# yinan-codes/Rossby-wave-ray-tracing

Hardware: AMD Instinct MI355X
Metric: ray-steps/sec (whole node), 10^6 rays RKF45; max |Δpos| vs CPU ref (higher is better)
Workload: dtype f64

## Files before the change

rossby-wave-ray-tracing_amd/csrc/ray_point.h:

```cpp
#ifndef RWRT_RAY_POINT_H
#define RWRT_RAY_POINT_H

#include <hip/hip_runtime.h>

#include <cmath>
#include <cstdint>

#include "rwrt.h"
#include "nproots.h"

#ifndef RARE
#define RARE(c) (c)
#endif

namespace rwrt {

constexpr double kPi = 3.14159265358979323846;
constexpr double kHalfPi = 0.5 * kPi;
constexpr double kTwoPi = 2.0 * kPi;
constexpr double kNaN = __builtin_nan("");

__device__ __forceinline__ void div2(double a1, double b1, double a2, double b2, double& qa,
                                     double& qb) {
  double dA, dB, rA, rB, eA, eB, nA, nB;
// ... 67 lines not shown
struct Field {
  const double* __restrict__ P;
  int W, H;
  double lon0, dlon, lat0, dlat;
};

struct Corners {
  const double* a;
  const double* b;
  const double* c;
  const double* d;
  double wa, wb, wc, wd;
  unsigned key_x, key_y;
  unsigned pa, pb, pc, pd;
  unsigned oa, ob, oc, od;
};

__device__ __forceinline__ Corners corners(const Field& F, double lon, double lat) {
  const double lons = py_mod_2pi_again(lon);
  double x, y;
  div2(lons - F.lon0, F.dlon, lat - F.lat0, F.dlat, x, y);
  const int ix = floor_i32(x), iy = floor_i32(y);
  const int x0 = clip(ix, F.W - 1), x1 = clip(inc_i32(ix), F.W - 1);
  const int y0 = clip(iy, F.H - 1), y1 = clip(inc_i32(iy), F.H - 1);
  const double sx = x - (double)x0, sy = y - (double)y0;
  const unsigned c0 = __umul24(x0, F.H), c1 = __umul24(x1, F.H);
  Corners k;
  k.pa = c0 + y1;
  k.pb = c1 + y1;
  k.pc = c0 + y0;
  k.pd = c1 + y0;
  k.oa = __umul24(k.pa, kNF);
  k.ob = __umul24(k.pb, kNF);
  k.oc = __umul24(k.pc, kNF);
  k.od = __umul24(k.pd, kNF);
  k.a = F.P + k.oa;
  k.b = F.P + k.ob;
  k.c = F.P + k.oc;
  k.d = F.P + k.od;
  k.wa = (1.0 - sx) * sy;
  k.wb = sx * sy;
  k.wc = (1.0 - sx) * (1.0 - sy);
// ... 136 lines not shown
```

rossby-wave-ray-tracing_amd/csrc/rwrt.hip:

```cpp

#include <hip/hip_runtime.h>

#include <cmath>
#include <cstdint>
#include <cstdlib>
#include <cstdio>
#include <cstring>
#include <mutex>
#include <string>
#include <type_traits>

#include "rwrt.h"
#include "nproots.h"

#ifdef RWRT_ANALYZE_HOT
__device__ __forceinline__ bool rwrt_rare_sink(bool c) {
  asm volatile("; rare %0" ::"s"(__builtin_amdgcn_ballot_w64(c)));
  return false;
}
#define RARE(c) rwrt_rare_sink(c)
#else
#define RARE(c) (c)
#endif
#ifdef RWRT_ANALYZE_MARK
// ... 64 lines not shown
  return (ab >= 0x1p-100 && ab <= 0x1p100) ? r : 0.0;
}
__device__ __forceinline__ double div_hw(double a, double b, double rb) {
  const double q = a * rb;
  const double rem = fma(-b, q, a);
  double r = copysign(fma(rem, rb, q), q);
  const double aa = fabs(a);
  const bool bad = !(aa < 0x1p600) | ((aa < 0x1p-900) & (aa != 0.0)) | (rb == 0.0);
  if (RARE(bad)) {
    asm volatile("");
    r = a / b;
  }
  return r;
}

__constant__ int kRefIndex[11] = {0, 1, 2, 3, 4, 5, 6, 7, 8, 9, 11};

struct StaticBG {
  static constexpr bool kTimeVarying = false;
  Field F;
  const char* img = nullptr;
  __device__ __forceinline__ void interp11(double lon, double lat, double, double g[11]) const {
    rwrt::interp11(F, py_mod_2pi(lon), lat, g);
  }
  __device__ __forceinline__ void interp4(double lon, double lat, double, double& fu, double& fv,
                                          double& fqx, double& fqy) const {
    rwrt::interp4(F, py_mod_2pi(lon), lat, fu, fv, fqx, fqy);
  }
};

struct PendingPoint {
  double lon, lat, t;
};
template <class BG>
__device__ __forceinline__ PendingPoint lookup_begin(const BG&, double lon, double lat, double t) {
  return PendingPoint{lon, lat, t};
}
template <class BG>
__device__ __forceinline__ void lookup_end(const BG& B, const PendingPoint& p, double g[11]) {
  B.interp11(p.lon, p.lat, p.t, g);
}

constexpr int kCacheChunks = 4 * 6;
constexpr int kCacheBytesPerWave = kCacheChunks * 64 * 16;
// ... 4 lines not shown
  typedef __attribute__((address_space(3))) char lds_char;
  unsigned b = (unsigned)(size_t)(lds_char*)wave_base;
  asm volatile("" : "+s"(b));
  return (char*)(lds_char*)(size_t)b;
}

__device__ __forceinline__ void lds_dma_wait() { asm volatile("s_waitcnt vmcnt(0)" ::: "memory"); }

constexpr int kCacheAhead = 1;
static_assert(kCacheAhead >= 0 && kCacheAhead < 4, "end() prologue waits for chunks 0-3 only");

constexpr unsigned kImgTile = 6 * 1024;
inline size_t cache_image_bytes(int64_t npts) { return (size_t)((npts + 63) / 64) * kImgTile; }
__device__ __forceinline__ unsigned img_offset(unsigned p) { return __umul24(p >> 6, kImgTile - 1024u) + p * 16u; }

__global__ void cache_image_kernel(Field F, char* __restrict__ img) {
  const int64_t n = (int64_t)F.W * F.H * 6;
  for (int64_t i = blockIdx.x * (int64_t)blockDim.x + threadIdx.x; i < n; i += (int64_t)gridDim.x * blockDim.x) {
    const unsigned p = (unsigned)(i / 6), q = (unsigned)(i - (int64_t)p * 6);
    const double2 v = reinterpret_cast<const double2*>(F.P + (size_t)p * kNF)[q];
    *reinterpret_cast<double2*>(img + img_offset(p) + q * 1024u) = v;
  }
}

struct CachedStaticBG {
  static constexpr bool kTimeVarying = false;
  Field F;
  const char* img;
  char* wave_base;
  const char* img_hi;
  unsigned lane16;
  mutable unsigned key_x, key_y;

  struct Pending {
    double wa, wb, wc, wd;
  };
  __device__ __forceinline__ const double2& chunk(int j, int q) const {
    return *reinterpret_cast<const double2*>(wave_base + (j * 6 + q) * 1024 + lane16);
  }
  __device__ __forceinline__ void refill(unsigned o0, unsigned o1, unsigned o2, unsigned o3) const {
    typedef __attribute__((address_space(3))) char lds_char;
    const unsigned l = (unsigned)(size_t)(lds_char*)wave_base;
    unsigned keep;
#define RWRT_REFILL_LO(O, LOFF)                                                  \
    "s_add_u32 m0, %[l], " #LOFF "\n\t"                                          \
    "s_nop 0\n\t"                                                               \
    "global_load_lds_dwordx4 %[" #O "], %[g0]\n\t"                              \
    "global_load_lds_dwordx4 %[" #O "], %[g0] offset:1024\n\t"                  \
    "global_load_lds_dwordx4 %[" #O "], %[g0] offset:2048\n\t"                  \
    "global_load_lds_dwordx4 %[" #O "], %[g0] offset:3072\n\t"
// ... 49 lines not shown
    if (k.key_x != key_x || k.key_y != key_y) {
      quad_refill(img_offset(k.pa), img_offset(k.pb), img_offset(k.pc), img_offset(k.pd), qa, qb);
      key_x = k.key_x;
      key_y = k.key_y;
    }
    return Pending{k.wa, k.wb, k.wc, k.wd};
  }
  __device__ __forceinline__ Pending begin(double lon, double lat) const {
    const Corners k = corners(F, py_mod_2pi(lon), lat);
    const bool miss = k.key_x != key_x || k.key_y != key_y;
    if (miss) {
      refill(img_offset(k.pa), img_offset(k.pb), img_offset(k.pc), img_offset(k.pd));
      key_x = k.key_x;
      key_y = k.key_y;
    }
    return Pending{k.wa, k.wb, k.wc, k.wd};
  }
  template <class Fill>
  __device__ __forceinline__ void end(const Pending& p, double g[11], Fill&& fill) const {
    asm volatile("s_waitcnt vmcnt(8)" ::: "memory");
    Corners k;
    k.wa = p.wa;
    k.wb = p.wb;
    k.wc = p.wc;
    k.wd = p.wd;
    constexpr int kAhead = kCacheAhead;
    double2 v[6][4];
#pragma unroll
    for (int q = 0; q <= kAhead; ++q)
#pragma unroll
      for (int j = 0; j < 4; ++j) v[q][j] = chunk(j, q);
// ... 10 lines not shown
        if (n == 4) lds_dma_wait();
#pragma unroll
        for (int j = 0; j < 4; ++j) v[n][j] = chunk(j, n);
      }
      __builtin_amdgcn_sched_barrier(0);
    }
  }
  __device__ __forceinline__ void interp4(double lon, double lat, double, double& fu, double& fv,
                                          double& fqx, double& fqy) const {
    rwrt::interp4(F, py_mod_2pi(lon), lat, fu, fv, fqx, fqy);
  }
};
__device__ __forceinline__ CachedStaticBG::Pending lookup_begin(const CachedStaticBG& B, double lon,
                                                                double lat, double) {
  return B.begin(lon, lat);
}
__device__ __forceinline__ void lookup_end(const CachedStaticBG& B,
                                           const CachedStaticBG::Pending& p, double g[11]) {
  B.end(p, g, [] {});
}
template <class Fill>
__device__ __forceinline__ void lookup_end(const CachedStaticBG& B, const CachedStaticBG::Pending& p,
                                           double g[11], Fill&& fill) {
  B.end(p, g, fill);
}
template <class BG, class Fill>
__device__ __forceinline__ void lookup_end(const BG& B, const typename std::decay<decltype(lookup_begin(
                                                            B, 0.0, 0.0, 0.0))>::type& p,
                                           double g[11], Fill&& fill) {
  fill();
// ... 694 lines not shown
}
__device__ __forceinline__ void ugvg(double fu, double fv, double fqx, double fqy,
                                     const KapTerms& w, double& ug, double& vg) {
  const double kap = w.kap, kap2 = w.kap2, denom = w.denom;
  double qu, qv;
  div2(((1.0 - kap2) * fqy) - ((2.0 * kap) * fqx), denom,
       ((2.0 * kap) * fqy) + ((1.0 - kap2) * fqx), denom, qu, qv);
  ug = fu + qu;
  vg = fv + qv;
}
__device__ __forceinline__ void ugvg(double fu, double fv, double fqx, double fqy,
                                     double k, double l, double& ug, double& vg) {
  ugvg(fu, fv, fqx, fqy, kap_terms(k, l), ug, vg);
}

__device__ __forceinline__ double rcp2(double d) {
  double r = __builtin_amdgcn_rcp(d);
  double e = fma(-d, r, 1.0);
  r = fma(r, e, r);
  e = fma(-d, r, 1.0);
  return fma(r, e, r);
}
__device__ __forceinline__ double qdiv(double n, double d, double r) {
  const double q = n * r;
  const double e = fma(-d, q, n);
  return __builtin_amdgcn_div_fixup(fma(e, r, q), d, n);
}
struct DivGuard {
  int nlo = 0, nhi = 0, dlo = 0, dhi = 0;
  __device__ __forceinline__ void num(double n) {
    const int e = __builtin_amdgcn_frexp_exp(n);
    nlo = ::min(nlo, e);
    nhi = ::max(nhi, e);
  }
  __device__ __forceinline__ void den(double d) {
    const int e = __builtin_amdgcn_frexp_exp(d);
    dlo = ::min(dlo, e);
    dhi = ::max(dhi, e);
  }
  __device__ __forceinline__ bool ok() const {
    return (nlo >= -899) & (nhi <= 600) & (dlo >= -99) & (dhi <= 100);
  }
// ... 65 lines not shown
  const double dzwn = (-kx) * ((fmux + kap * fmvx) + qk);
  const double dmwn = (-kx) * ((fmuy + kap * fmvy) + ql);
  const double damp1 = qdiv(2.0 * ((fmux + fmvy) + kap * (fmvx + fmuy)), kw.kap1, kw.rk1, G);
  const double damp2 = qdiv(2.0 * (kap * (fmqxx - fmqyy) + (kap2 - 1.0) * fmqxy), kw.denom, kw.rden, G);
  const double damp3 = (-2.0 * s) * fmv;
  const double damp = (damp1 + damp2) + damp3;
  const double rR = rcp2(kREarth);
  dy[0] = qdiv(ug, kREarth, rR, G);
  dy[1] = qdiv(vg * c, kREarth, rR, G);
  dy[2] = qdiv(dzwn, kREarth, rR, G);
  dy[3] = qdiv(dmwn, kREarth, rR, G);
  dy[4] = qdiv(damp * amp, kREarth, rR, G);
  return G.ok() & (M.m == 1.0);
}

__device__ __forceinline__ bool rhs_tail_fast_pair(const double g[11], const Merc& M, double s, double c,
                                                   double tn, double kx, const KapTermsR& kw, DivGuard G,
                                                   double amp, bool up, double& dA, double& dB, double& dC,
                                                   double& ug, double& vg) {
  const double fu = g[F_U], fv = g[F_V];
  const double rc = rcp2(c);
  const double fmuy = g[F_UY] + tn * fu, fmvy = g[F_VY] + tn * fv;
  const double fmqx = g[F_QX], fmqy = g[F_QY] * c, fmqxx = g[F_QXX];
  const double fmqyx = g[F_QXY] * c, fmqxy = fmqyx;
  const double fmqyy = ((g[F_QYY] * c) - (g[F_QY] * s)) * c;
  const double kap = kw.kap, kap2 = kw.kap2;
  const double fmu = qdiv(fu, c, rc, G), fmv = qdiv(fv, c, rc, G);
  const double fmux = qdiv(g[F_UX], c, rc, G), fmvx = qdiv(g[F_VX], c, rc, G);
  ug = fmu + qdiv(((1.0 - kap2) * fmqy) - ((2.0 * kap) * fmqx), kw.denom, kw.rden, G);
  vg = fmv + qdiv(((2.0 * kap) * fmqy) + ((1.0 - kap2) * fmqx), kw.denom, kw.rden, G);
// ... 1 lines not shown
  const double ql = qdiv(kap * fmqxy - fmqyy, kw.kk, kw.rkk, G);
  const double dzwn = (-kx) * ((fmux + kap * fmvx) + qk);
  const double dmwn = (-kx) * ((fmuy + kap * fmvy) + ql);
  const double damp1 = qdiv(2.0 * ((fmux + fmvy) + kap * (fmvx + fmuy)), kw.kap1, kw.rk1, G);
  const double damp2 = qdiv(2.0 * (kap * (fmqxx - fmqyy) + (kap2 - 1.0) * fmqxy), kw.denom, kw.rden, G);
  const double damp3 = (-2.0 * s) * fmv;
  const double damp = (damp1 + damp2) + damp3;
  const double rR = rcp2(kREarth);
  const double vgc = vg * c;
  dA = qdiv(up ? vgc : ug, kREarth, rR, G);
  dB = qdiv(up ? dmwn : dzwn, kREarth, rR, G);
  dC = qdiv(damp * amp, kREarth, rR, G);
  return G.ok() & (M.m == 1.0);
}

template <class BG>
__device__ __forceinline__ void ray_rhs(const BG& B, double t, const double* y, double* dy,
                                        double* aux = nullptr) {
  const double lon = y[0], lat = y[1], kx = y[2];
  const bool bad = fabs(lat) >= kHalfPi || fabs(y[3]) >= 100.0;
  const double ky = bad ? kNaN : y[3], amp = y[4];
  double g[11];
  MARK("r_entry");
  const auto trig = np_math::nm_sincostan_begin(lat);
  MARK("r_trig_begin");
  double s, c;
  DivGuard G;
  KapTermsR kw;
  const auto pending = lookup_begin(B, lon, lat, t);
  MARK("r_lookup_begin");
  double tn;
  np_math::nm_sincostan_end(lat, trig, s, c, tn);
  MARK("r_trig_end");
  __builtin_amdgcn_sched_barrier(0);
  lookup_end(B, pending, g, [&] { kw = kap_terms_r(kx, ky, G); MARK("r_kap"); });
  MARK("r_lookup_end");
  const Merc M = merc_factors(lat, c, s);
  double ug, vg;
  if (RARE(!rhs_tail_fast(g, M, s, c, tn, kx, kw, G, amp, dy, ug, vg))) {
    asm volatile("");
    rhs_tail_ieee(g, M, s, c, tn, kx, ky, amp, dy, ug, vg);
  }
  MARK("r_tail");
  if (aux) {
    aux[0] = ug;
    aux[1] = vg;
    aux[2] = bad ? kNaN : c;
  }
}

#ifndef RWRT_TEAM_SINORCOS
#define RWRT_TEAM_SINORCOS 1
#endif

template <class Lookup>
__device__ __forceinline__ void ray_rhs_f32(Lookup&& lookup, const double* y, double* dy, double* aux) {
  const double lat = y[1];
  const bool bad = fabs(lat) >= kHalfPi || fabs(y[3]) >= 100.0;
  const float fnan = __builtin_nanf("");
  const float kx = (float)y[2], ky = bad ? fnan : (float)y[3], amp = (float)y[4];
  float g[11];
  lookup(g);
  if (!(fabs(lat) <= kHalfPi)) {
// ... 592 lines not shown
__global__ void mercator_kernel(Field F, int64_t n, const double* __restrict__ lon,
                                const double* __restrict__ lat, double* __restrict__ out) {
  nm_stage<NM_SINCOS | NM_TAN>();
  for (int64_t i = blockIdx.x * (int64_t)blockDim.x + threadIdx.x; i < n;
       i += (int64_t)gridDim.x * blockDim.x) {
    const double la = lat[i];
    double g[11], o[12];
    interp11(F, py_mod_2pi(lon[i]), la, g);
    const Merc M = merc_factors(la, k_cos(la), k_sin(la));
    mercator12(g, M, k_tan(la), o);
#pragma unroll
    for (int q = 0; q < 12; ++q) out[q * n + i] = o[q];
  }
}

__global__ void rhs_kernel(Field F, int64_t n, const double* __restrict__ y,
                           double* __restrict__ dydt) {
  nm_stage<NM_SINCOS | NM_TAN>();
  for (int64_t i = blockIdx.x * (int64_t)blockDim.x + threadIdx.x; i < n;
       i += (int64_t)gridDim.x * blockDim.x) {
    double yy[5], d[5];
#pragma unroll
    for (int v = 0; v < 5; ++v) yy[v] = y[v * n + i];
    ray_rhs(StaticBG{F}, 0.0, yy, d);
#pragma unroll
    for (int v = 0; v < 5; ++v) dydt[v * n + i] = d[v];
  }
}

__global__ void attempt_kernel(Field F, int64_t n, const double* __restrict__ y,
                               const double* __restrict__ f, const double* __restrict__ h,
                               double rtol, double atol, double* __restrict__ Kout,
                               double* __restrict__ ynew, double* __restrict__ err) {
  nm_stage<NM_SINCOS | NM_TAN>();
  const RayProblem P{StaticBG{F}};
  for (int64_t i = blockIdx.x * (int64_t)blockDim.x + threadIdx.x; i < n;
       i += (int64_t)gridDim.x * blockDim.x) {
    double yy[5], ff[5], yn[5], k6[5];
#pragma unroll
// ... 527 lines not shown
  using type = BlockVaryingBG<T>;
};

template <class BG, class LBG, bool kTrace, bool kReplica, bool kPair = false>
__device__ __forceinline__ void run_rays(const RunArgs<BG>& a, const LBG& lbg, char* smem, int64_t hw) {
  using RayProblem = RayProblemT<LBG>;
  const RayProblem P{lbg};
  const bool writer = kReplica ? (threadIdx.x & 63u) == 0 : kPair ? (threadIdx.x & 63u) < 32u : true;
  Lane<RayProblem, KStore> L;
  L.K.p = reinterpret_cast<double*>(smem) + threadIdx.x;
  L.K.stride = 256;
  int64_t ray = -1, nacc = 0, nrej = 0;
  double* rows = nullptr;
  int32_t it = 0, nanrow = 0, wpos = 0;
  double prev_lon = 0.0, prev_lat = 0.0, cos_prev = 0.0;
  constexpr bool kHandoff = std::is_same<LBG, CachedStaticBG>::value && !kReplica && !kPair && !kTrace;
  bool handoff = false;
  __builtin_amdgcn_s_setprio(1);
  for (;;) {
    if (ray < 0) {
      int64_t w;
      if (kReplica) {
        if (hw < 0) break;
        w = hw;
        hw = -1;
      } else if (kPair) {
        int64_t w0 = 0;
        if ((threadIdx.x & 63u) < 32u) w0 = a.n_heavy + atomicAdd(&a.queue[1], 1);
        w = __shfl(w0, (int)(threadIdx.x & 31u));
      } else {
        w = a.n_heavy + atomicAdd(&a.queue[1], 1);
// ... 139 lines not shown
      if (q < nq) {
        CachedStaticBG QB = lbg;
        QB.key_x = QB.key_y = ~0u;
        QuadRole R;
        R.role = threadIdx.x & 3;
        R.odd = (R.role & 1) != 0;
        R.high = (R.role & 2) != 0;
        KQuad K{reinterpret_cast<double*>(smem) + threadIdx.x};
        quad_run<false>(a, QB, R, K, qray, qrows, y, f, aux, qt, qhabs, qhs, qnacc, qnrej, 0, qnanrow, qit,
                        qplon, qplat, qcos, (qflags & 1) != 0, (qflags & 2) != 0, 0);
      }
    }
  }
}

template <class BG, bool kTrace = false>
__global__ void __launch_bounds__(256, 1) __attribute__((aligned(RWRT_RUN_ALIGN)))
rk45_run_kernel(RunArgs<BG> a) {
  nm_stage<NM_ALL>();
  constexpr int kKBytes = 5 * 5 * 256 * 8;
  __shared__ __attribute__((aligned(16))) char smem[kKBytes + LaneBG<BG>::kLdsBytes];
  if constexpr (std::is_same<BG, StaticBG>::value) {
    const int lb = (int)blockIdx.x;
#ifdef RWRT_ANALYZE_QUAD
    if (true) {
#else
    if (RARE(lb < a.heavy_blocks)) {
#endif
      __builtin_amdgcn_s_setprio(1);
      quad_rays<kTrace>(a, smem + kKBytes, reinterpret_cast<double*>(smem), lb);
      return;
    }
  }
// ... 4 lines not shown
      using BBG = typename TvBlock<BG>::type;
      run_rays<BG, BBG, false, true>(a, BBG::make(a.B, smem + kKBytes), smem, w);
      return;
    }
  }
  if constexpr (std::is_same<BG, VaryingBG<double>>::value) {
#ifdef RWRT_ANALYZE_PAIR
    if (true) {
#else
    if (a.B.half) {
#endif
      run_rays<BG, PairVaryingBG64, false, false, true>(a, PairVaryingBG64::make(a.B, smem + kKBytes), smem, -1);
      return;
    }
  }
  run_rays<BG, typename LaneBG<BG>::type, kTrace, false>(a, LaneBG<BG>::make(a.B, smem + kKBytes), smem, -1);
}

__global__ void frozen_flag_kernel(const double* __restrict__ state, int64_t nray,
                                   uint8_t* __restrict__ frozen, int32_t* __restrict__ tail_from = nullptr,
                                   int32_t it_begin = 0, int32_t it_end = 0) {
  for (int64_t i = blockIdx.x * (int64_t)blockDim.x + threadIdx.x; i < nray;
       i += (int64_t)gridDim.x * blockDim.x) {
    double sum = state[i];
#pragma unroll
    for (int v = 1; v < 5; ++v) sum = sum + state[v * nray + i];
    const bool frz = isnan(sum / 5.0);
    frozen[i] = frz ? 1 : 0;
    if (tail_from) tail_from[i] = frz ? it_begin : it_end;
  }
}
// ... 114 lines not shown
    case 26: r = np_math::nm_cos(a); break;
    case 27: r = np_math::nm_tan(a); break;
    case 28: r = np_math::nm_pow(a, b); break;
    case 29: r = np_math::nm_rcp14(a); break;
    case 30: { double sn, cs, tn; k_sincostan(a, sn, cs, tn); r = sn; } break;
    case 31: { double sn, cs, tn; k_sincostan(a, sn, cs, tn); r = cs; } break;
    case 32: { double sn, cs, tn; k_sincostan(a, sn, cs, tn); r = tn; } break;
    case 33: r = k_pow(a, b); break;
    case 34: r = qdiv(a, b, rcp2(b)); break;
    case 35: {
      DivGuard G;
      G.num(a);
      G.den(b);
      r = G.ok() ? 1.0 : 0.0;
    } break;
    default: r = kNaN; break;
  }
  out[i] = r;
}

__device__ __forceinline__ bool rhs_bad(const double* y) {
  return fabs(y[1]) >= kHalfPi || fabs(y[3]) >= 100.0;
}

struct Rk4Args {
  Field F;
  const char* img;
  int64_t nray;
  double dt, cut_off;
  int32_t nt, it_begin, it_end;
// ... 342 lines not shown
rwrt_status ctx_flags(rwrt_ctx* c, int64_t nray) {
  if ((size_t)nray <= c->cap) return RWRT_OK;
  if (c->flags) {
    if ((c->used && hipEventSynchronize(c->done) != hipSuccess) || hipFree(c->flags) != hipSuccess)
      return check_launch("releasing the context's frozen-ray flags");
    c->flags = nullptr;
    c->cap = 0;
  }
  const size_t cap = ((size_t)nray + 4095) & ~(size_t)4095;
  if (hipMalloc(reinterpret_cast<void**>(&c->flags), cap) != hipSuccess)
    return fail(RWRT_ERR_HIP, "frozen-ray flag allocation failed%s");
  c->cap = cap;
  return RWRT_OK;
}

rwrt_status ctx_image(rwrt_ctx* c, const Field& F, hipStream_t stream, const char** out) {
  const size_t need = cache_image_bytes((int64_t)F.W * F.H);
  if (need > c->img_cap) {
    if (c->img) {
      if ((c->used && hipEventSynchronize(c->done) != hipSuccess) || hipFree(c->img) != hipSuccess)
        return check_launch("releasing the context's cache image");
      c->img = nullptr;
      c->img_cap = 0;
    }
    if (hipMalloc(reinterpret_cast<void**>(&c->img), need) != hipSuccess)
      return fail(RWRT_ERR_HIP, "cache image allocation failed%s");
    c->img_cap = need;
  }
  hipLaunchKernelGGL(cache_image_kernel, dim3(grid_for((int64_t)F.W * F.H * 6, 256)), dim3(256), 0, stream,
                     F, c->img);
  *out = c->img;
  return check_launch("cache_image_kernel");
}

template <class BG> int& ctx_blocks(rwrt_ctx* c);
template <> int& ctx_blocks<StaticBG>(rwrt_ctx* c) { return c->blocks_static; }
template <> int& ctx_blocks<VaryingBG<float>>(rwrt_ctx* c) { return c->blocks_f32; }
template <> int& ctx_blocks<VaryingBG<double>>(rwrt_ctx* c) { return c->blocks_f64; }
template <> int& ctx_blocks<VaryingBGA32>(rwrt_ctx* c) { return c->blocks_a32; }

template <class BG>
int ctx_persistent_blocks(rwrt_ctx* c) {
  int& b = ctx_blocks<BG>(c);
  if (!b) b = persistent_blocks_on<BG>(c->ncu);
  return b;
}
// ... 65 lines not shown
  const int64_t need = (nray - n_heavy + block_rays - 1) / block_rays;
  if (blocks > need) blocks = need;
  RunArgs<BG> a{B, nray, p->rtol, p->atol, p->min_step, p->cut_off, p->nt, it_begin, it_end,
                d_tbound, d_order, d_state, d_count, d_nanrow, d_out, d_work,
                n_heavy, 0, haversine_cut(p->cut_off), nullptr};
  a.row_slot = d_row_slot;
  a.handoff = handoff;
  if (rwrt_status s = ctx_flags(ctx, nray)) return s;
  a.frozen = ctx->flags;
  if (rwrt_status s = ctx_begin(ctx, st, [&] {
        hipLaunchKernelGGL(frozen_flag_kernel, dim3(grid_for(nray, 256)), dim3(256), 0, st, d_state, nray,
                           ctx->flags, d_tail_from, it_begin, it_end);
      }))
    return s;
  if constexpr (std::is_same<BG, StaticBG>::value) {
    if (rwrt_status s = ctx_image(ctx, B.F, st, &a.B.img)) return s;
  }
  a.heavy_blocks = (int32_t)team_blocks;
  a.quad_per_wave = quad_per_wave;
  if constexpr (std::is_same<BG, StaticBG>::value) {
    a.trace = ctx->trace;
    a.trace_cap = ctx->trace ? ctx->trace_cap : 0;
  }
  if (nray > n_heavy || team_blocks) {
    const int64_t grid = team_blocks + (nray > n_heavy ? blocks : 0);
    if (a.trace && std::is_same<BG, StaticBG>::value) {
      if constexpr (std::is_same<BG, StaticBG>::value)
        hipLaunchKernelGGL((rk45_run_kernel<BG, true>), dim3((unsigned)grid), dim3(256), 0, st, a);
    } else {
      hipLaunchKernelGGL(rk45_run_kernel<BG>, dim3((unsigned)grid), dim3(256), 0, st, a);
    }
    if (rwrt_status s = check_launch("rk45_run_kernel")) return s;
  }
  if (d_tail_from)
    hipLaunchKernelGGL(frozen_tail_kernel<BG>, dim3((unsigned)((nray + kFillThreads - 1) / kFillThreads)),
                       dim3(kFillThreads), 0, ctx->side, a, d_tail_row);
  else
    hipLaunchKernelGGL(frozen_fill_kernel<BG>, dim3((unsigned)((nray + kFillThreads - 1) / kFillThreads)),
                       dim3(kFillThreads), 0, ctx->side, a);
  if (rwrt_status s = check_launch(d_tail_from ? "frozen_tail_kernel" : "frozen_fill_kernel")) return s;
  return ctx_end(ctx, st);
}

template <class T>
rwrt_status make_varying(const rwrt_grid* g, const rwrt_background* b, VaryingBG<T>& B) {
// ... 341 lines not shown
  Field F;
  if (rwrt_status s = make_field(g, d_packed, F)) return s;
  if (n < 0 || (n > 0 && (!d_lon || !d_lat || !d_out))) return fail(RWRT_ERR_ARG, "bad point arrays%s");
  if (n == 0) return RWRT_OK;
  hipLaunchKernelGGL(mercator_kernel, dim3(grid_for(n, 256)), dim3(256), 0, (hipStream_t)stream, F,
                     n, d_lon, d_lat, d_out);
  return check_launch("mercator_kernel");
}

rwrt_status rwrt_rhs(const rwrt_grid* g, const double* d_packed, int64_t n, const double* d_y,
                     double* d_dydt, void* stream) {
  Field F;
  if (rwrt_status s = make_field(g, d_packed, F)) return s;
  if (n < 0 || (n > 0 && (!d_y || !d_dydt))) return fail(RWRT_ERR_ARG, "bad state arrays%s");
  if (n == 0) return RWRT_OK;
  hipLaunchKernelGGL(rhs_kernel, dim3(grid_for(n, 256)), dim3(256), 0, (hipStream_t)stream, F, n,
                     d_y, d_dydt);
  return check_launch("rhs_kernel");
}

rwrt_status rwrt_dp54_attempt(const rwrt_grid* g, const double* d_packed, int64_t n,
                              const double* d_y, const double* d_f, const double* d_h,
                              double rtol, double atol, double* d_K, double* d_ynew,
                              double* d_err, void* stream) {
  Field F;
  if (rwrt_status s = make_field(g, d_packed, F)) return s;
  if (n < 0 || (n > 0 && (!d_y || !d_f || !d_h || !d_K || !d_ynew || !d_err)))
    return fail(RWRT_ERR_ARG, "bad attempt arrays%s");
  if (n == 0) return RWRT_OK;
  hipLaunchKernelGGL(attempt_kernel, dim3(grid_for(n, 256)), dim3(256), 0, (hipStream_t)stream, F,
                     n, d_y, d_f, d_h, rtol, atol, d_K, d_ynew, d_err);
  return check_launch("attempt_kernel");
}
// ... 276 lines not shown
                          double* d_out, void* stream) {
  if (ncol <= 0 || nt < 1 || !d_y0 || !d_teval || !d_out) return fail(RWRT_ERR_ARG, "bad KAT arguments%s");
  const dim3 grid(grid_for(ncol, 64)), block(64);
  hipStream_t s = (hipStream_t)stream;
  switch (kind) {
    case 0: hipLaunchKernelGGL(kat_kernel<KatLinear>, grid, block, 0, s, ncol, d_y0, nt, d_teval, rtol, atol, min_step, d_out); break;
    case 1: hipLaunchKernelGGL(kat_kernel<KatExp>, grid, block, 0, s, ncol, d_y0, nt, d_teval, rtol, atol, min_step, d_out); break;
    case 2: hipLaunchKernelGGL(kat_kernel<KatLorenz>, grid, block, 0, s, ncol, d_y0, nt, d_teval, rtol, atol, min_step, d_out); break;
    default: return fail(RWRT_ERR_ARG, "unknown KAT kind%s");
  }
  return check_launch("kat_kernel");
}

rwrt_status rwrt_selftest_math(int32_t kind, int64_t n, const double* d_x, const double* d_y,
                               double* d_out, void* stream) {
  if (n < 0 || kind < 0 || kind > 37 || (n > 0 && (!d_x || !d_out)))
    return fail(RWRT_ERR_ARG, "bad selftest arguments%s");
  if (kind >= 17 && kind <= 22)
    return fail(RWRT_ERR_ARG, "selftest kinds 17-22 are retired%s");
  if (n == 0) return RWRT_OK;
  if (kind >= 36) {
    if (!d_y) return fail(RWRT_ERR_ARG, "selftest kinds 36/37 need d_y%s");
    hipLaunchKernelGGL(jump_verdict_kernel, dim3(grid_for(n, 256)), dim3(256), 0, (hipStream_t)stream, kind,
                       n, d_x, d_y, d_out, haversine_cut(0.05));
    return check_launch("jump_verdict_kernel");
  }
  hipLaunchKernelGGL(math_kernel, dim3(grid_for(n, 256)), dim3(256), 0, (hipStream_t)stream, kind,
                     n, d_x, d_y, d_out);
  return check_launch("math_kernel");
}

rwrt_status rwrt_host_fill_rows(double* dst, int64_t nrows, int64_t ncol, int64_t ld,
                                const double* prev, const double* src, int64_t nsrc,
                                int64_t ld_src, const int64_t* cols) {
  if (nrows < 0 || ncol < 0 || nsrc < 0 || nsrc > ncol || ld < ncol || ld_src < nsrc)
    return fail(RWRT_ERR_ARG, "bad rwrt_host_fill_rows shape%s");
// ... 34 lines not shown
```

rossby-wave-ray-tracing_amd/engine.py:

```python
import os

import numpy as np
import torch

import _hip as H
from constants import rearth as R_EARTH
from launch_rows import deliver

F64 = torch.float64


def grid_of(lon, lat, ncol):
    lon = np.asarray(lon, np.float64)
    lat = np.asarray(lat, np.float64)
    return H.Grid(int(ncol), len(lat), float(lon[0]), float(lon[1] - lon[0]),
                  float(lat[0]), float(lat[1] - lat[0]))


def t_eval_of(nt, tstep, ttotal=None):
    t = np.arange(nt) * np.float64(tstep)
    if ttotal is not None and t[-1] > ttotal:
        t[-1] = ttotal
    return t

# ... 713 lines not shown
    te = torch.as_tensor(t_eval, dtype=F64, device=device).contiguous()
    nv, ncol = y0.shape
    out = torch.empty((ncol, len(t_eval), nv), dtype=F64, device=device)
    H.check(H.load().rwrt_kat_rk45(int(kind), ncol, H.dptr(y0), len(t_eval), H.dptr(te),
                                   float(max(rtol, 100 * np.finfo(np.float64).eps)), float(atol),
                                   float(min_step), H.dptr(out), H.stream(y0.device)))
    return out.permute(1, 2, 0)


MATH_KINDS = {"sin": 0, "cos": 1, "tan": 2, "pow": 3, "atan2": 4, "mod": 5, "sqrt": 6,
              "div": 7, "floor": 8, "sincos_sin": 9, "sincos_cos": 10, "div_rearth": 11,
              "fmod": 12, "mod2pi": 13, "mod2pi_twice": 14, "div_hw": 15, "floor_i32": 16,
              "div2_first": 23,
              "div2_second": 24, "nm_sin": 25, "nm_cos": 26, "nm_tan": 27, "nm_pow": 28,
              "nm_rcp14": 29, "k_sin": 30, "k_cos": 31, "k_tan": 32, "k_pow": 33,
              "qdiv": 34, "qdiv_exact_range": 35, "jump_verdict_fast": 36, "jump_verdict_exact": 37}


def selftest_math(name, x, y=None, device="cuda"):
    H.require_gpu()
    x = torch.as_tensor(np.asarray(x, np.float64), device=device).contiguous()
    yt = None if y is None else torch.as_tensor(np.asarray(y, np.float64), device=device).contiguous()
    out = torch.empty_like(x)
    H.check(H.load().rwrt_selftest_math(MATH_KINDS[name], x.numel(), H.dptr(x), H.dptr(yt),
                                        H.dptr(out), H.stream(x.device)))
    return out.cpu().numpy()
```

Before: 3.977 billion.

## Add lean RHS tier gated by background-field exponent range scan

```diff
diff --git a/rossby-wave-ray-tracing_amd/csrc/ray_point.h b/rossby-wave-ray-tracing_amd/csrc/ray_point.h
--- a/rossby-wave-ray-tracing_amd/csrc/ray_point.h
+++ b/rossby-wave-ray-tracing_amd/csrc/ray_point.h
@@ -105,18 +105,22 @@
   unsigned key_x, key_y;
   unsigned pa, pb, pc, pd;
   unsigned oa, ob, oc, od;
+  double dx, dy;
 };
 
 __device__ __forceinline__ Corners corners(const Field& F, double lon, double lat) {
   const double lons = py_mod_2pi_again(lon);
   double x, y;
-  div2(lons - F.lon0, F.dlon, lat - F.lat0, F.dlat, x, y);
+  const double dx = lons - F.lon0, dy = lat - F.lat0;
+  div2(dx, F.dlon, dy, F.dlat, x, y);
   const int ix = floor_i32(x), iy = floor_i32(y);
   const int x0 = clip(ix, F.W - 1), x1 = clip(inc_i32(ix), F.W - 1);
   const int y0 = clip(iy, F.H - 1), y1 = clip(inc_i32(iy), F.H - 1);
   const double sx = x - (double)x0, sy = y - (double)y0;
   const unsigned c0 = __umul24(x0, F.H), c1 = __umul24(x1, F.H);
   Corners k;
+  k.dx = dx;
+  k.dy = dy;
   k.pa = c0 + y1;
   k.pb = c1 + y1;
   k.pc = c0 + y0;
diff --git a/rossby-wave-ray-tracing_amd/csrc/rwrt.hip b/rossby-wave-ray-tracing_amd/csrc/rwrt.hip
--- a/rossby-wave-ray-tracing_amd/csrc/rwrt.hip
+++ b/rossby-wave-ray-tracing_amd/csrc/rwrt.hip
@@ -102,12 +102,25 @@
   return r;
 }
 
+__device__ __forceinline__ double rcp2(double d) {
+  double r = __builtin_amdgcn_rcp(d);
+  double e = fma(-d, r, 1.0);
+  r = fma(r, e, r);
+  e = fma(-d, r, 1.0);
+  return fma(r, e, r);
+}
+__device__ __forceinline__ double qdiv(double n, double d, double r) {
+  const double q = n * r;
+  const double e = fma(-d, q, n);
+  return __builtin_amdgcn_div_fixup(fma(e, r, q), d, n);
+}
 __constant__ int kRefIndex[11] = {0, 1, 2, 3, 4, 5, 6, 7, 8, 9, 11};
 
 struct StaticBG {
   static constexpr bool kTimeVarying = false;
   Field F;
   const char* img = nullptr;
+  const int* range = nullptr;
   __device__ __forceinline__ void interp11(double lon, double lat, double, double g[11]) const {
     rwrt::interp11(F, py_mod_2pi(lon), lat, g);
   }
@@ -116,6 +129,8 @@
     rwrt::interp4(F, py_mod_2pi(lon), lat, fu, fv, fqx, fqy);
   }
 };
+
+struct LeanStaticBG : StaticBG {};
 
 struct PendingPoint {
   double lon, lat, t;
@@ -150,13 +165,76 @@
 inline size_t cache_image_bytes(int64_t npts) { return (size_t)((npts + 63) / 64) * kImgTile; }
 __device__ __forceinline__ unsigned img_offset(unsigned p) { return __umul24(p >> 6, kImgTile - 1024u) + p * 16u; }
 
-__global__ void cache_image_kernel(Field F, char* __restrict__ img) {
+constexpr int kExpBias = 2048;
+constexpr int kRangeInts = 4;
+struct ExpRange {
+  int a = 0, b = 0, bad = 0;
+  __device__ __forceinline__ void see(double v) {
+    const int e = __builtin_amdgcn_frexp_exp(v);
+    const bool fin = fabs(v) < __builtin_inf();
+    if (fin && v != 0.0) {
+      a = ::max(a, kExpBias - e);
+      b = ::max(b, kExpBias + e);
+    }
+    bad |= fin ? 0 : 1;
+  }
+  __device__ __forceinline__ void publish(int* range) {
+#pragma unroll
+    for (int d = 32; d >= 1; d >>= 1) {
+      a = ::max(a, __shfl_xor(a, d));
+      b = ::max(b, __shfl_xor(b, d));
+      bad |= __shfl_xor(bad, d);
+    }
+    if ((threadIdx.x & 63u) == 0) {
+      if (a) atomicMax(range + 0, a);
+      if (b) atomicMax(range + 1, b);
+      if (bad) atomicMax(range + 2, 1);
+    }
+  }
+};
+
+constexpr int kLeafLo = -100;
+constexpr int kLeafAmpHi = 100;
+constexpr int kLeafKLo = -7, kLeafKHi = 19;
+constexpr int kBgLo = -250, kBgHi = 200;
+constexpr int kStepLo = -30, kStepHi = 2;
+constexpr int kOriginLonHi = 3, kOriginLatHi = 1;
+__device__ __forceinline__ bool cell_leaf_ok(double dx, double dy) {
+  const int ex = __builtin_amdgcn_frexp_exp(dx), ey = __builtin_amdgcn_frexp_exp(dy);
+  return ::min(ex, ey) >= kLeafLo;
+}
+__device__ __forceinline__ bool bg_lean(const int* range, const Field& F) {
+  if (!range) return false;
+  const int a = range[0], b = range[1], bad = range[2];
+  const int es = __builtin_amdgcn_frexp_exp(F.dlon), et = __builtin_amdgcn_frexp_exp(F.dlat);
+  const bool ok = bad == 0 && (a == 0 || kExpBias - a >= kBgLo) && (b == 0 || b - kExpBias <= kBgHi) &&
+                  ::min(es, et) >= kStepLo && ::max(es, et) <= kStepHi &&
+                  __builtin_amdgcn_frexp_exp(F.lon0) <= kOriginLonHi &&
+                  __builtin_amdgcn_frexp_exp(F.lat0) <= kOriginLatHi;
+  return __builtin_amdgcn_readfirstlane((int)ok) != 0;
+}
+
+__global__ void cache_image_kernel(Field F, char* __restrict__ img, int* __restrict__ range) {
   const int64_t n = (int64_t)F.W * F.H * 6;
+  ExpRange R;
   for (int64_t i = blockIdx.x * (int64_t)blockDim.x + threadIdx.x; i < n; i += (int64_t)gridDim.x * blockDim.x) {
     const unsigned p = (unsigned)(i / 6), q = (unsigned)(i - (int64_t)p * 6);
     const double2 v = reinterpret_cast<const double2*>(F.P + (size_t)p * kNF)[q];
     *reinterpret_cast<double2*>(img + img_offset(p) + q * 1024u) = v;
-  }
+    R.see(v.x);
+    R.see(v.y);
+  }
+  R.publish(range);
+}
+__global__ void bg_range_kernel(Field F, int* __restrict__ range) {
+  const int64_t n = (int64_t)F.W * F.H * 6;
+  ExpRange R;
+  for (int64_t i = blockIdx.x * (int64_t)blockDim.x + threadIdx.x; i < n; i += (int64_t)gridDim.x * blockDim.x) {
+    const double2 v = reinterpret_cast<const double2*>(F.P)[i];
+    R.see(v.x);
+    R.see(v.y);
+  }
+  R.publish(range);
 }
 
 struct CachedStaticBG {
@@ -170,6 +248,7 @@
 
   struct Pending {
     double wa, wb, wc, wd;
+    bool cell_ok;
   };
   __device__ __forceinline__ const double2& chunk(int j, int q) const {
     return *reinterpret_cast<const double2*>(wave_base + (j * 6 + q) * 1024 + lane16);
@@ -249,7 +328,7 @@
       key_x = k.key_x;
       key_y = k.key_y;
     }
-    return Pending{k.wa, k.wb, k.wc, k.wd};
+    return Pending{k.wa, k.wb, k.wc, k.wd, cell_leaf_ok(k.dx, k.dy)};
   }
   template <class Fill>
   __device__ __forceinline__ void end(const Pending& p, double g[11], Fill&& fill) const {
@@ -290,6 +369,16 @@
 __device__ __forceinline__ CachedStaticBG::Pending lookup_begin(const CachedStaticBG& B, double lon,
                                                                 double lat, double) {
   return B.begin(lon, lat);
+}
+struct LeanCachedStaticBG : CachedStaticBG {};
+__device__ __forceinline__ CachedStaticBG::Pending lookup_begin(const LeanCachedStaticBG& B, double lon,
+                                                                double lat, double) {
+  return B.begin(lon, lat);
+}
+template <class Fill>
+__device__ __forceinline__ void lookup_end(const LeanCachedStaticBG& B, const CachedStaticBG::Pending& p,
+                                           double g[11], Fill&& fill) {
+  B.end(p, g, fill);
 }
 __device__ __forceinline__ void lookup_end(const CachedStaticBG& B,
                                            const CachedStaticBG::Pending& p, double g[11]) {
@@ -1014,18 +1103,13 @@
   ugvg(fu, fv, fqx, fqy, kap_terms(k, l), ug, vg);
 }
 
-__device__ __forceinline__ double rcp2(double d) {
-  double r = __builtin_amdgcn_rcp(d);
-  double e = fma(-d, r, 1.0);
-  r = fma(r, e, r);
-  e = fma(-d, r, 1.0);
-  return fma(r, e, r);
-}
-__device__ __forceinline__ double qdiv(double n, double d, double r) {
-  const double q = n * r;
-  const double e = fma(-d, q, n);
-  return __builtin_amdgcn_div_fixup(fma(e, r, q), d, n);
-}
+__device__ __forceinline__ bool leaf_ok(bool cell_ok, double lat, double k, double l, double amp) {
+  const int ea = __builtin_amdgcn_frexp_exp(amp), ek = __builtin_amdgcn_frexp_exp(k);
+  const int lo = ::min(::min(__builtin_amdgcn_frexp_exp(lat), __builtin_amdgcn_frexp_exp(l)), ea);
+  return cell_ok && lo >= kLeafLo && ea <= kLeafAmpHi &&
+         (unsigned)(ek - kLeafKLo) <= (unsigned)(kLeafKHi - kLeafKLo);
+}
+constexpr double kRcpREarth = 0x1.510fa3eaca281p-23;
 struct DivGuard {
   int nlo = 0, nhi = 0, dlo = 0, dhi = 0;
   __device__ __forceinline__ void num(double n) {
@@ -1121,6 +1205,48 @@
   return G.ok() & (M.m == 1.0);
 }
 
+__device__ __forceinline__ KapTermsR kap_terms_lean(double k, double l) {
+  KapTermsR w;
+  w.kap = qdiv(l, k, rcp2(k));
+  w.kap2 = w.kap * w.kap;
+  w.kap1 = 1.0 + w.kap2;
+  w.kk = (k * k) * w.kap1;
+  w.denom = w.kk * w.kap1;
+  w.rkk = rcp2(w.kk);
+  w.rk1 = rcp2(w.kap1);
+  w.rden = rcp2(w.denom);
+  return w;
+}
+__device__ __forceinline__ void rhs_tail_lean(const double g[11], double s, double c, double tn, double kx,
+                                              const KapTermsR& kw, double amp, double* dy, double& ug,
+                                              double& vg) {
+  const double fu = g[F_U], fv = g[F_V];
+  const double rc = rcp2(c);
+  const double fmu = qdiv(fu, c, rc), fmv = qdiv(fv, c, rc);
+  const double fmux = qdiv(g[F_UX], c, rc), fmvx = qdiv(g[F_VX], c, rc);
+  const double fmuy = g[F_UY] + tn * fu, fmvy = g[F_VY] + tn * fv;
+  const double fmqx = g[F_QX], fmqy = g[F_QY] * c, fmqxx = g[F_QXX];
+  const double fmqyx = g[F_QXY] * c, fmqxy = fmqyx;
+  const double fmqyy = ((g[F_QYY] * c) - (g[F_QY] * s)) * c;
+  const double kap = kw.kap, kap2 = kw.kap2;
+  ug = fmu + qdiv(((1.0 - kap2) * fmqy) - ((2.0 * kap) * fmqx), kw.denom, kw.rden);
+  vg = fmv + qdiv(((2.0 * kap) * fmqy) + ((1.0 - kap2) * fmqx), kw.denom, kw.rden);
+  const double qk = qdiv(kap * fmqxx - fmqyx, kw.kk, kw.rkk);
+  const double ql = qdiv(kap * fmqxy - fmqyy, kw.kk, kw.rkk);
+  const double dzwn = (-kx) * ((fmux + kap * fmvx) + qk);
+  const double dmwn = (-kx) * ((fmuy + kap * fmvy) + ql);
+  const double damp1 = qdiv(2.0 * ((fmux + fmvy) + kap * (fmvx + fmuy)), kw.kap1, kw.rk1);
+  const double damp2 = qdiv(2.0 * (kap * (fmqxx - fmqyy) + (kap2 - 1.0) * fmqxy), kw.denom, kw.rden);
+  const double damp3 = (-2.0 * s) * fmv;
+  const double damp = (damp1 + damp2) + damp3;
+  const double rR = kRcpREarth;
+  dy[0] = qdiv(ug, kREarth, rR);
+  dy[1] = qdiv(vg * c, kREarth, rR);
+  dy[2] = qdiv(dzwn, kREarth, rR);
+  dy[3] = qdiv(dmwn, kREarth, rR);
+  dy[4] = qdiv(damp * amp, kREarth, rR);
+}
+
 __device__ __forceinline__ bool rhs_tail_fast_pair(const double g[11], const Merc& M, double s, double c,
                                                    double tn, double kx, const KapTermsR& kw, DivGuard G,
                                                    double amp, bool up, double& dA, double& dB, double& dC,
@@ -1152,9 +1278,22 @@
   return G.ok() & (M.m == 1.0);
 }
 
-template <class BG>
-__device__ __forceinline__ void ray_rhs(const BG& B, double t, const double* y, double* dy,
-                                        double* aux = nullptr) {
+template <class BG> struct HasLean : std::false_type {};
+template <> struct HasLean<LeanStaticBG> : std::true_type {};
+template <> struct HasLean<LeanCachedStaticBG> : std::true_type {};
+__device__ __forceinline__ bool pending_cell_ok(const LeanCachedStaticBG&, const CachedStaticBG::Pending& p) {
+  return p.cell_ok;
+}
+__device__ __forceinline__ bool pending_cell_ok(const LeanStaticBG& B, const PendingPoint& p) {
+  return cell_leaf_ok(py_mod_2pi_again(py_mod_2pi(p.lon)) - B.F.lon0, p.lat - B.F.lat0);
+}
+template <class BG, class P>
+__device__ __forceinline__ bool pending_cell_ok(const BG&, const P&) {
+  return false;
+}
+
+template <bool kLean, class BG>
+__device__ __forceinline__ void ray_rhs_tier(const BG& B, double t, const double* y, double* dy, double* aux) {
   const double lon = y[0], lat = y[1], kx = y[2];
   const bool bad = fabs(lat) >= kHalfPi || fabs(y[3]) >= 100.0;
   const double ky = bad ? kNaN : y[3], amp = y[4];
@@ -1171,11 +1310,22 @@
   np_math::nm_sincostan_end(lat, trig, s, c, tn);
   MARK("r_trig_end");
   __builtin_amdgcn_sched_barrier(0);
-  lookup_end(B, pending, g, [&] { kw = kap_terms_r(kx, ky, G); MARK("r_kap"); });
+  lookup_end(B, pending, g, [&] {
+    if constexpr (kLean) kw = kap_terms_lean(kx, ky);
+    else kw = kap_terms_r(kx, ky, G);
+    MARK("r_kap");
+  });
   MARK("r_lookup_end");
   const Merc M = merc_factors(lat, c, s);
   double ug, vg;
-  if (RARE(!rhs_tail_fast(g, M, s, c, tn, kx, kw, G, amp, dy, ug, vg))) {
+  if constexpr (kLean) {
+    const bool ok = leaf_ok(pending_cell_ok(B, pending), lat, kx, ky, amp) && M.m == 1.0;
+    rhs_tail_lean(g, s, c, tn, kx, kw, amp, dy, ug, vg);
+    if (RARE(!ok)) {
+      asm volatile("");
+      rhs_tail_ieee(g, M, s, c, tn, kx, ky, amp, dy, ug, vg);
+    }
+  } else if (RARE(!rhs_tail_fast(g, M, s, c, tn, kx, kw, G, amp, dy, ug, vg))) {
     asm volatile("");
     rhs_tail_ieee(g, M, s, c, tn, kx, ky, amp, dy, ug, vg);
   }
@@ -1185,6 +1335,11 @@
     aux[1] = vg;
     aux[2] = bad ? kNaN : c;
   }
+}
+template <class BG>
+__device__ __forceinline__ void ray_rhs(const BG& B, double t, const double* y, double* dy,
+                                        double* aux = nullptr) {
+  ray_rhs_tier<HasLean<BG>::value>(B, t, y, dy, aux);
 }
 
 #ifndef RWRT_TEAM_SINORCOS
@@ -1807,15 +1962,17 @@
   }
 }
 
-__global__ void rhs_kernel(Field F, int64_t n, const double* __restrict__ y,
+__global__ void rhs_kernel(Field F, const int* __restrict__ range, int64_t n, const double* __restrict__ y,
                            double* __restrict__ dydt) {
   nm_stage<NM_SINCOS | NM_TAN>();
+  const bool lean = bg_lean(range, F);
   for (int64_t i = blockIdx.x * (int64_t)blockDim.x + threadIdx.x; i < n;
        i += (int64_t)gridDim.x * blockDim.x) {
     double yy[5], d[5];
 #pragma unroll
     for (int v = 0; v < 5; ++v) yy[v] = y[v * n + i];
-    ray_rhs(StaticBG{F}, 0.0, yy, d);
+    if (lean) ray_rhs(LeanStaticBG{{F}}, 0.0, yy, d);
+    else ray_rhs(StaticBG{F}, 0.0, yy, d);
 #pragma unroll
     for (int v = 0; v < 5; ++v) dydt[v * n + i] = d[v];
   }
@@ -2373,7 +2530,7 @@
   double* rows = nullptr;
   int32_t it = 0, nanrow = 0, wpos = 0;
   double prev_lon = 0.0, prev_lat = 0.0, cos_prev = 0.0;
-  constexpr bool kHandoff = std::is_same<LBG, CachedStaticBG>::value && !kReplica && !kPair && !kTrace;
+  constexpr bool kHandoff = std::is_base_of<CachedStaticBG, LBG>::value && !kReplica && !kPair && !kTrace;
   bool handoff = false;
   __builtin_amdgcn_s_setprio(1);
   for (;;) {
@@ -2543,9 +2700,15 @@
   }
 }
 
-template <class BG, bool kTrace = false>
+template <class BG, bool kTrace = false, bool kLean = false>
 __global__ void __launch_bounds__(256, 1) __attribute__((aligned(RWRT_RUN_ALIGN)))
 rk45_run_kernel(RunArgs<BG> a) {
+  static_assert(!kLean || std::is_same<BG, StaticBG>::value, "the lean tier is the static state's");
+#ifndef RWRT_ANALYZE_HOT
+  if constexpr (std::is_same<BG, StaticBG>::value) {
+    if (bg_lean(a.B.range, a.B.F) != kLean) return;
+  }
+#endif
   nm_stage<NM_ALL>();
   constexpr int kKBytes = 5 * 5 * 256 * 8;
   __shared__ __attribute__((aligned(16))) char smem[kKBytes + LaneBG<BG>::kLdsBytes];
@@ -2580,7 +2743,11 @@
       return;
     }
   }
-  run_rays<BG, typename LaneBG<BG>::type, kTrace, false>(a, LaneBG<BG>::make(a.B, smem + kKBytes), smem, -1);
+  if constexpr (kLean)
+    run_rays<BG, LeanCachedStaticBG, kTrace, false>(a, LeanCachedStaticBG{LaneBG<BG>::make(a.B, smem + kKBytes)}, smem,
+                                                    -1);
+  else
+    run_rays<BG, typename LaneBG<BG>::type, kTrace, false>(a, LaneBG<BG>::make(a.B, smem + kKBytes), smem, -1);
 }
 
 __global__ void frozen_flag_kernel(const double* __restrict__ state, int64_t nray,
@@ -2725,6 +2892,19 @@
       G.den(b);
       r = G.ok() ? 1.0 : 0.0;
     } break;
+    case 40: {
+      const int leaf = (int)b;
+      double v[6] = {1.0, 1.0, 0.5, 3.0, 2.0, 1.0};
+      if (leaf >= 0 && leaf < 6) v[leaf] = a;
+      const bool masked = fabs(v[2]) >= kHalfPi || fabs(v[4]) >= 100.0;
+      r = leaf_ok(cell_leaf_ok(v[0], v[1]), v[2], v[3], masked ? kNaN : v[4], v[5]) ? 1.0 : 0.0;
+    } break;
+    case 41: r = rcp2(a); break;
+    case 42: r = kRcpREarth; break;
+    case 43: {
+      const int e = __builtin_amdgcn_frexp_exp(a);
+      r = (a == 0.0 || (fabs(a) < __builtin_inf() && e >= kBgLo && e <= kBgHi)) ? 1.0 : 0.0;
+    } break;
     default: r = kNaN; break;
   }
   out[i] = r;
@@ -3097,8 +3277,9 @@
   return RWRT_OK;
 }
 
-rwrt_status ctx_image(rwrt_ctx* c, const Field& F, hipStream_t stream, const char** out) {
-  const size_t need = cache_image_bytes((int64_t)F.W * F.H);
+rwrt_status ctx_image(rwrt_ctx* c, const Field& F, hipStream_t stream, const char** out,
+                      const int** range = nullptr) {
+  const size_t image = cache_image_bytes((int64_t)F.W * F.H), need = image + kRangeInts * sizeof(int);
   if (need > c->img_cap) {
     if (c->img) {
       if ((c->used && hipEventSynchronize(c->done) != hipSuccess) || hipFree(c->img) != hipSuccess)
@@ -3110,9 +3291,13 @@
       return fail(RWRT_ERR_HIP, "cache image allocation failed%s");
     c->img_cap = need;
   }
+  int* r = reinterpret_cast<int*>(c->img + image);
+  if (hipMemsetAsync(r, 0, kRangeInts * sizeof(int), stream) != hipSuccess)
+    return check_launch("hipMemsetAsync(exponent range)");
   hipLaunchKernelGGL(cache_image_kernel, dim3(grid_for((int64_t)F.W * F.H * 6, 256)), dim3(256), 0, stream,
-                     F, c->img);
+                     F, c->img, r);
   *out = c->img;
+  if (range) *range = r;
   return check_launch("cache_image_kernel");
 }
 
@@ -3208,7 +3393,7 @@
       }))
     return s;
   if constexpr (std::is_same<BG, StaticBG>::value) {
-    if (rwrt_status s = ctx_image(ctx, B.F, st, &a.B.img)) return s;
+    if (rwrt_status s = ctx_image(ctx, B.F, st, &a.B.img, &a.B.range)) return s;
   }
   a.heavy_blocks = (int32_t)team_blocks;
   a.quad_per_wave = quad_per_wave;
@@ -3219,10 +3404,14 @@
   if (nray > n_heavy || team_blocks) {
     const int64_t grid = team_blocks + (nray > n_heavy ? blocks : 0);
     if (a.trace && std::is_same<BG, StaticBG>::value) {
-      if constexpr (std::is_same<BG, StaticBG>::value)
+      if constexpr (std::is_same<BG, StaticBG>::value) {
         hipLaunchKernelGGL((rk45_run_kernel<BG, true>), dim3((unsigned)grid), dim3(256), 0, st, a);
+        hipLaunchKernelGGL((rk45_run_kernel<BG, true, true>), dim3((unsigned)grid), dim3(256), 0, st, a);
+      }
     } else {
       hipLaunchKernelGGL(rk45_run_kernel<BG>, dim3((unsigned)grid), dim3(256), 0, st, a);
+      if constexpr (std::is_same<BG, StaticBG>::value)
+        hipLaunchKernelGGL((rk45_run_kernel<BG, false, true>), dim3((unsigned)grid), dim3(256), 0, st, a);
     }
     if (rwrt_status s = check_launch("rk45_run_kernel")) return s;
   }
@@ -3594,9 +3783,23 @@
   if (rwrt_status s = make_field(g, d_packed, F)) return s;
   if (n < 0 || (n > 0 && (!d_y || !d_dydt))) return fail(RWRT_ERR_ARG, "bad state arrays%s");
   if (n == 0) return RWRT_OK;
-  hipLaunchKernelGGL(rhs_kernel, dim3(grid_for(n, 256)), dim3(256), 0, (hipStream_t)stream, F, n,
-                     d_y, d_dydt);
-  return check_launch("rhs_kernel");
+  hipStream_t st = (hipStream_t)stream;
+  int* range = nullptr;
+  if (hipMallocAsync(reinterpret_cast<void**>(&range), kRangeInts * sizeof(int), st) != hipSuccess)
+    return fail(RWRT_ERR_HIP, "exponent-range allocation failed%s");
+  rwrt_status rs = RWRT_OK;
+  if (hipMemsetAsync(range, 0, kRangeInts * sizeof(int), st) != hipSuccess) {
+    rs = check_launch("hipMemsetAsync(exponent range)");
+  } else {
+    hipLaunchKernelGGL(bg_range_kernel, dim3(grid_for((int64_t)F.W * F.H * 6, 256)), dim3(256), 0, st, F, range);
+    rs = check_launch("bg_range_kernel");
+  }
+  if (rs == RWRT_OK) {
+    hipLaunchKernelGGL(rhs_kernel, dim3(grid_for(n, 256)), dim3(256), 0, st, F, range, n, d_y, d_dydt);
+    rs = check_launch("rhs_kernel");
+  }
+  if (hipFreeAsync(range, st) != hipSuccess && rs == RWRT_OK) rs = check_launch("hipFreeAsync(exponent range)");
+  return rs;
 }
 
 rwrt_status rwrt_dp54_attempt(const rwrt_grid* g, const double* d_packed, int64_t n,
@@ -3903,12 +4106,12 @@
 
 rwrt_status rwrt_selftest_math(int32_t kind, int64_t n, const double* d_x, const double* d_y,
                                double* d_out, void* stream) {
-  if (n < 0 || kind < 0 || kind > 37 || (n > 0 && (!d_x || !d_out)))
+  if (n < 0 || kind < 0 || kind > 43 || kind == 38 || kind == 39 || (n > 0 && (!d_x || !d_out)))
     return fail(RWRT_ERR_ARG, "bad selftest arguments%s");
   if (kind >= 17 && kind <= 22)
     return fail(RWRT_ERR_ARG, "selftest kinds 17-22 are retired%s");
   if (n == 0) return RWRT_OK;
-  if (kind >= 36) {
+  if (kind == 36 || kind == 37) {
     if (!d_y) return fail(RWRT_ERR_ARG, "selftest kinds 36/37 need d_y%s");
     hipLaunchKernelGGL(jump_verdict_kernel, dim3(grid_for(n, 256)), dim3(256), 0, (hipStream_t)stream, kind,
                        n, d_x, d_y, d_out, haversine_cut(0.05));
diff --git a/rossby-wave-ray-tracing_amd/engine.py b/rossby-wave-ray-tracing_amd/engine.py
--- a/rossby-wave-ray-tracing_amd/engine.py
+++ b/rossby-wave-ray-tracing_amd/engine.py
@@ -751,7 +751,8 @@
               "div2_first": 23,
               "div2_second": 24, "nm_sin": 25, "nm_cos": 26, "nm_tan": 27, "nm_pow": 28,
               "nm_rcp14": 29, "k_sin": 30, "k_cos": 31, "k_tan": 32, "k_pow": 33,
-              "qdiv": 34, "qdiv_exact_range": 35, "jump_verdict_fast": 36, "jump_verdict_exact": 37}
+              "qdiv": 34, "qdiv_exact_range": 35, "jump_verdict_fast": 36, "jump_verdict_exact": 37,
+              "leaf_guard": 40, "rcp2": 41, "rcp_rearth_literal": 42, "bg_window": 43}
 
 
 def selftest_math(name, x, y=None, device="cuda"):
```

Measured after the change: 4.040 billion (median of 6 runs). +1.6%, better.
